# Anima-Lab/MaskDiT

Measured on AMD Instinct MI355X. Metric: training img/sec MaskDiT-XL/2 256 mask=0.5 bs=1024, higher is better.
Workload: dtype bf16; 1 GPU; DiT-XL/2 ImageNet256-latent [32x32x4], mask_ratio=0.5, mae_loss_coef=0.1, sample(moments)+class-dropout+fwd+bwd+grad-allreduce+AdamW+EMA, random-init (de-zeroed) weights; global_batch=1024, per_gpu_batch=1024, micro_batch=1024, accum=1, parallelism=dp1

## Files before the change

### include/maskdit_hip.h

```cpp
#ifndef MASKDIT_HIP_H
#define MASKDIT_HIP_H

#include <stdint.h>

#ifdef __cplusplus
extern "C" {
#endif

typedef void* mdt_stream_t;
typedef uint16_t mdt_bf16;

const char* mdt_last_error(void);
#define MDT_ABI_VERSION 4
int mdt_version(void);
int mdt_set_tuning(const char* key, int value);
int mdt_lds_poison(void* sink4, mdt_stream_t stream);
int mdt_nt8o_report(unsigned* abort_code, unsigned long long* stats16, int reset);
int mdt_nt8o_stamps(unsigned long long* host192);


enum mdt_epilogue {
  MDT_EPI_BF16 = 0,
  MDT_EPI_F32 = 1,
  MDT_EPI_GELU = 2,
// ... 8 lines not shown
  const mdt_bf16* B; int ldb;
  int M, N, K;
  const float* bias;
  int epi;
  mdt_bf16* out; int ldo;
  mdt_bf16* out2; int ldo2;
  float* outf; int ldof;
  const float* res; int ldres;
  const float* gate; int gate_ld; int rows_per_sample;
  const mdt_bf16* aux; int ldaux;
  int k_splits;
  float* colsum;
} mdt_gemm_nt_args;
int mdt_gemm_nt(const mdt_gemm_nt_args* a, mdt_stream_t stream);

typedef struct {
  const mdt_bf16* A; int lda;
  const mdt_bf16* B; int ldb;
  int M, N1, N2;
  float* C; int ldc;
  int n1_valid, n2_valid;
  int splits;
  float* colsum_a;
} mdt_gemm_tn_args;
int mdt_gemm_tn(const mdt_gemm_tn_args* a, mdt_stream_t stream);


int mdt_attn_fwd(const mdt_bf16* qkv, mdt_bf16* out, float* lse, int B, int L, int H, int hd, int L_valid,
                 mdt_stream_t stream);
int mdt_attn_bwd(const mdt_bf16* qkv, const mdt_bf16* out, const mdt_bf16* dout, const float* lse,
                 float* delta, mdt_bf16* dqkv, int B, int L, int H, int hd, int L_valid, mdt_stream_t stream);


int mdt_ln_modulate_fwd(const float* x, const float* shift, const float* scale, int mod_ld,
                        int rows_per_sample, mdt_bf16* xn, float* stats, int M, int D,
                        mdt_stream_t stream);
int mdt_ln_modulate_fwd_res(const float* xres, const mdt_bf16* y, const float* gate, int gate_ld, const float* shift,
                            const float* scale, int mod_ld, int rows_per_sample, float* x, mdt_bf16* xn, float* stats,
                            int M, int D, mdt_stream_t stream);
int mdt_ln_modulate_bwd(const mdt_bf16* dxn, const float* x, const float* stats, const float* scale,
                        int mod_ld, int rows_per_sample, float* dx, int accumulate, float* dshift,
                        float* dscale, int dmod_ld, int M, int D, mdt_stream_t stream);
int mdt_ln_modulate_bwd_gate(const mdt_bf16* dxn, const float* x, const float* stats, const float* scale,
                             int mod_ld, int rows_per_sample, float* dx, int accumulate, float* dshift,
                             float* dscale, int dmod_ld, int M, int D, const mdt_bf16* y, const float* gate,
                             int gate_ld, mdt_bf16* dys, float* dgate, int dgate_ld, float* dbias,
                             mdt_stream_t stream);
int mdt_gate_bwd(const float* dx, const mdt_bf16* y, const float* gate, int mod_ld,
// ... 204 lines not shown
```

### maskdit_amd/_lib.py

```python
from __future__ import annotations

import ctypes as C
import os
import subprocess

_HERE = os.path.dirname(os.path.abspath(__file__))
LIB_PATH = os.environ.get('MASKDIT_HIP_LIB') or os.path.join(_HERE, 'libmaskdit_hip.so')
CSRC = os.path.join(_HERE, 'csrc')

vp = C.c_void_p
i32 = C.c_int
i64 = C.c_long
f32 = C.c_float

EPI_BF16, EPI_F32, EPI_GELU, EPI_SILU, EPI_GATE_RES, EPI_DGELU, EPI_DSILU = range(7)


class GemmNTArgs(C.Structure):
    _fields_ = [('A', vp), ('lda', i32), ('B', vp), ('ldb', i32), ('M', i32), ('N', i32), ('K', i32),
                ('bias', vp), ('epi', i32), ('out', vp), ('ldo', i32), ('out2', vp), ('ldo2', i32),
                ('outf', vp), ('ldof', i32), ('res', vp), ('ldres', i32), ('gate', vp), ('gate_ld', i32),
                ('rows_per_sample', i32), ('aux', vp), ('ldaux', i32), ('k_splits', i32), ('colsum', vp)]


class GemmTNArgs(C.Structure):
    _fields_ = [('A', vp), ('lda', i32), ('B', vp), ('ldb', i32), ('M', i32), ('N1', i32), ('N2', i32),
                ('C', vp), ('ldc', i32), ('n1_valid', i32), ('n2_valid', i32), ('splits', i32), ('colsum_a', vp)]


class GemmF32Args(C.Structure):
    _fields_ = [('A', vp), ('lda', i64), ('B', vp), ('ldb', i64), ('b_kmajor', i32), ('M', i32), ('N', i32), ('K', i32),
                ('bias', vp), ('epi', i32), ('out', vp), ('ldo', i64), ('res', vp), ('ldres', i64), ('gate', vp),
                ('gate_ld', i64), ('rows_per_sample', i32), ('batch', i32), ('heads', i32),
                ('a_stride_b', i64), ('a_stride_h', i64), ('b_stride_b', i64), ('b_stride_h', i64),
                ('o_stride_b', i64), ('o_stride_h', i64)]


F32EPI_NONE, F32EPI_GELU, F32EPI_SILU, F32EPI_GATE_RES = range(4)


class GemmF32TNArgs(C.Structure):
    _fields_ = [('A', vp), ('lda', i64), ('B', vp), ('ldb', i64), ('M', i32), ('N1', i32), ('N2', i32), ('C', vp), ('ldc', i64),
                ('accumulate', i32), ('batch', i32), ('heads', i32),
                ('a_stride_b', i64), ('a_stride_h', i64), ('b_stride_b', i64), ('b_stride_h', i64),
                ('c_stride_b', i64), ('c_stride_h', i64), ('ws', vp), ('ws_floats', i64)]


_PROTOS = {
    'mdt_gemm_nt': [C.POINTER(GemmNTArgs)],
    'mdt_gemm_tn': [C.POINTER(GemmTNArgs)],
# ... 62 lines not shown
    'mdt_attn_f32_bwd': [vp, vp, vp, i64, vp, i32, i32, i32, i32],
    'mdt_ln_modulate_bwd_f32': [vp, vp, vp, i32, i32, vp, i32, vp, vp, i32, vp, i32, i32],
    'mdt_gate_bwd_f32': [vp, vp, vp, i32, i32, vp, vp, i32, i32, i32],
    'mdt_gate_res_f32': [vp, vp, vp, i32, i32, vp, i32, i32],
    'mdt_gelu_f32': [vp, vp, i64],
    'mdt_gelu_bwd_f32': [vp, vp, vp, i64],
    'mdt_silu_bwd_f32': [vp, vp, vp, i64],
}
_PLAIN = {
    'mdt_graph_begin': [vp],
    'mdt_graph_end': [vp, C.POINTER(vp)],
    'mdt_graph_launch': [vp, vp],
    'mdt_graph_destroy': [vp],
    'mdt_event_create': [C.POINTER(vp)],
    'mdt_event_record': [vp, vp],
    'mdt_event_elapsed_ms': [vp, vp, C.POINTER(f32)],
    'mdt_event_destroy': [vp],
    'mdt_set_tuning': [C.c_char_p, i32],
    'mdt_nt8o_report': [C.POINTER(C.c_uint32), C.POINTER(C.c_uint64), i32],
    'mdt_nt8o_stamps': [C.POINTER(C.c_uint64)],
    'mdt_attn_f32_ws_floats': [i32, i32, i32, i32],
    'mdt_gn_stats_ordered_ws_floats': [i32, i32],
    'mdt_gemm_f32_tn_ws_floats': [i32, i32, i32, i32],
    'mdt_colsum_f32_ws_floats': [i32, i32],
    'mdt_attn_f32_bwd_ws_floats': [i32, i32, i32, i32],
}
EXPORTED = sorted(list(_PROTOS) + list(_PLAIN) + ['mdt_last_error', 'mdt_version'])
ABI_VERSION = 4


class MaskDiTLibError(RuntimeError):
    pass


def source_hash() -> str:
    import glob
    import hashlib
    h = hashlib.sha256()
    root = os.path.dirname(os.path.abspath(__file__))
    files = sorted(glob.glob(os.path.join(root, 'csrc', '*.hip')) + glob.glob(os.path.join(root, 'csrc', '*.h')) +
                   glob.glob(os.path.join(root, '..', 'include', '*.h')))
    for f in files:
        h.update(os.path.basename(f).encode())
        h.update(open(f, 'rb').read())
    return h.hexdigest()[:16]

# ... 60 lines not shown
```

### maskdit_amd/csrc/gemm.hip

```cpp
#include "common.h"
#include "../../include/maskdit_hip.h"

#include "gemm_common.h"

#define BM 128
#define BN 128
#define BK 64
#define STAGE_BYTES 32768

__global__ __launch_bounds__(256, 2) void gemm_nt_kernel(NTParams p) {
  __shared__ __attribute__((aligned(16))) char smem[2 * STAGE_BYTES];
  const int tid = threadIdx.x;
  const int lane = tid & 63;
  const int wave = __builtin_amdgcn_readfirstlane(tid >> 6);
  const int wr = wave >> 1, wc = wave & 1;

  const int tiles_m = (p.M + BM - 1) / BM, tiles_n = p.N / BN;
  int tm, tn;
  tile_coords(xcd_remap(blockIdx.x, gridDim.x), tiles_m, tiles_n, tm, tn);
  const int m0 = tm * BM, n0 = tn * BN;

  const int lr = lane >> 3, cpos = lane & 7;
  const int gch = cpos ^ lr;
  const bf16* a_src[4];
// ... 259 lines not shown
      }
      if (w4 < 0.97 * w8 && w4 < 1e29) return launch_gemm_nt8(p, nf4, 1, (hipStream_t)stream);
      if (w8 < 1e29) return launch_gemm_nt8(p, nf8, 2, (hipStream_t)stream);
    }
    p.epi &= 0xff;
  }
  p.epi &= 0xff;
  int tiles = cdiv(a->M, BM) * (a->N / BN);
  int ks = 1;
  if (a->k_splits > 1) {
    MDT_REQUIRE(a->epi == MDT_EPI_F32 && a->out == nullptr, "gemm_nt: k_splits needs MDT_EPI_F32 without a bf16 output");
    MDT_REQUIRE(a->ldof == a->N, "gemm_nt: k_splits needs a dense outf (ldof == N)");
    ks = a->k_splits < a->K / BK ? a->k_splits : a->K / BK;
    if (hipMemsetAsync(a->outf, 0, sizeof(float) * (size_t)a->M * a->N, (hipStream_t)stream) != hipSuccess) {
      mdt_set_error("gemm_nt: clearing the split-K accumulator failed");
      return MDT_ERR_LAUNCH;
    }
  }
  p.k_splits = ks;
  hipLaunchKernelGGL(gemm_nt_kernel, dim3(tiles, ks), dim3(256), 0, (hipStream_t)stream, p);
  return mdt_check_launch("gemm_nt");
}

extern "C" int mdt_gemm_tn(const mdt_gemm_tn_args* a, mdt_stream_t stream) {
  MDT_REQUIRE(a && a->A && a->B && a->C, "gemm_tn: null operand");
  MDT_REQUIRE(a->M > 0 && a->M % BK == 0, "gemm_tn: M must be a positive multiple of 64");
  MDT_REQUIRE(a->N1 > 0 && a->N2 > 0, "gemm_tn: empty output");
  MDT_REQUIRE(a->lda % 8 == 0 && a->ldb % 8 == 0, "gemm_tn: lda/ldb must be multiples of 8");
  MDT_REQUIRE(a->lda >= cdiv(a->N1, BM) * BM && a->ldb >= cdiv(a->N2, BN) * BN,
              "gemm_tn: operand rows must be padded to a multiple of 128 columns");
  MDT_REQUIRE(((uintptr_t)a->A & 15) == 0 && ((uintptr_t)a->B & 15) == 0, "gemm_tn: operands must be 16-byte aligned");
  TNParams p;
  p.A = (const bf16*)a->A; p.lda = a->lda; p.B = (const bf16*)a->B; p.ldb = a->ldb;
  p.M = a->M; p.N1 = a->N1; p.N2 = a->N2; p.C = a->C; p.ldc = a->ldc;
  p.n1_valid = a->n1_valid > 0 ? a->n1_valid : a->N1;
  p.n2_valid = a->n2_valid > 0 ? a->n2_valid : a->N2;
  const int tn_variant = mdt_get_tuning_int(MDT_TUNE_GEMM_TN_VARIANT);
  if (tn_variant != 1 && p.n1_valid == a->N1 && p.n2_valid == a->N2 && a->N1 % 128 == 0 && a->N2 % 128 == 0 &&
      a->M % 32 == 0 && a->M >= 8192 && (long)a->N1 * a->N2 >= 256L * 1024) {
    int cs_done = 0;
    int rc = launch_gemm_tn8(p.A, p.lda, p.B, p.ldb, p.M, p.N1, p.N2, p.C, p.ldc, (hipStream_t)stream, a->colsum_a, &cs_done, a->splits);
    if (rc == MDT_OK && a->colsum_a && !cs_done) rc = mdt_colsum_bf16(a->A, a->lda, a->colsum_a, a->M, a->N1, stream);
    return rc;
  }
  if (a->colsum_a) {
    int rc = mdt_colsum_bf16(a->A, a->lda, a->colsum_a, a->M, a->N1, stream);
    if (rc != MDT_OK) return rc;
  }
  int tiles = cdiv(a->N1, BM) * cdiv(a->N2, BN);
  int ksteps = a->M / BK;
  int splits = a->splits;
  if (splits <= 0) {
    splits = 2048 / tiles;
    if (splits > ksteps / 8) splits = ksteps / 8;
    if (splits < 1) splits = 1;
  }
  if (splits > ksteps) splits = ksteps;
  p.ksteps_per_split = cdiv(ksteps, splits);
  splits = cdiv(ksteps, p.ksteps_per_split);
  p.splits = splits;
  hipLaunchKernelGGL(gemm_tn_kernel, dim3(tiles * splits), dim3(256), 0, (hipStream_t)stream, p);
  return mdt_check_launch("gemm_tn");
}
```

### maskdit_amd/csrc/gemm_common.h

```cpp
#pragma once
#include "common.h"
#include "../../include/maskdit_hip.h"

#define GROUP_M 8

struct NTParams {
  const bf16* A; int lda;
  const bf16* B; int ldb;
  int M, N, K;
  const float* bias;
  int epi;
  bf16* out; int ldo;
  bf16* out2; int ldo2;
  float* outf; int ldof;
  const float* res; int ldres;
  const float* gate; int gate_ld; int rows_per_sample;
  const bf16* aux; int ldaux;
  int k_splits;
  int group_m;
  float* colsum;
  int conv_ho_log2, conv_up, conv_c;
  float* gn_sums; int gn_cpg_log2;
};

// ... 129 lines not shown
  nt_load_bias<CW>(p, n, bias);
  nt_epilogue_prefetch<CW>(p, m, n, d);
  nt_epilogue_finish<CW>(p, m, n, v, bias, d, csum);
}

template <int CW> __device__ __forceinline__ void nt_colsum_flush(const NTParams& p, int n, float* csum, int lane) {
#pragma unroll
  for (int q = 0; q < CW; ++q) {
    float s = csum[q];
    s += __shfl_xor(s, 4, 64);
    s += __shfl_xor(s, 8, 64);
    s += __shfl_xor(s, 16, 64);
    s += __shfl_xor(s, 32, 64);
    if (lane < 4) atomic_add_f32(p.colsum + n + q, s);
  }
}

int launch_gemm_nt8(const NTParams& p, int nf, int wr, hipStream_t stream);
int nt8_num_cus();
int nt8_max_nf(int epi);
bool nt8o_eligible(const NTParams& p);
int launch_gemm_nt8o(const NTParams& p, int nl, int dbg, hipStream_t stream);
int launch_gemm_tn8(const bf16* A, int lda, const bf16* B, int ldb, int M, int N1, int N2, float* C, int ldc,
                    hipStream_t stream, float* colsum_a = nullptr, int* colsum_done = nullptr, int forced_splits = 0);
```

### maskdit_amd/csrc/gemm_tn8.hip

```cpp
#include "gemm_common.h"

template <int YF> struct TN8Cfg {
  static constexpr int NSLOT = YF == 6 ? 5 : 6;
  static constexpr int SLOT_BYTES = YF == 6 ? 28672 : 24576;
  static constexpr int TY = 32 * YF;
  static constexpr int UNROLL = YF == 6 ? 10 : 6;
};

__device__ __forceinline__ int tn8_swz(int r) { return ((r & 3) | (((r >> 3) & 1) << 2)) << 1; }
__device__ __forceinline__ int tn8_swz2(int r) { return (((r >> 1) & 1) | (((r >> 3) & 1) << 1)) << 1; }

struct TN8Params {
  const bf16* X; int ldx;
  const bf16* Y; int ldy;
  int NX, NY;
  float* C; int ldc;
  int swap;
  int slots_total;
  int slots_per_split;
  int tiles_x, tiles_y;
  float* colsum_x;
  int group_x;
  int dbg;
  int long_k, long_len;
};

template <int OFF> __device__ __forceinline__ bf16x4 tn8_tr_read(unsigned addr) {
  static_assert(OFF >= 0 && OFF < 65536, "ds offset field is 16 bits");
  short4_t v;
  asm volatile("ds_read_b64_tr_b16 %0, %1 offset:%2" : "=v"(v) : "v"(addr), "n"(OFF));
  return __builtin_bit_cast(bf16x4, v);
}

template <int N> __device__ __forceinline__ void tn8_wait() {
  static_assert(N >= 0 && N < 64, "vmcnt is 6 bits");
  asm volatile("; MDT_CHK hand_wait" ::: "memory");
  __builtin_amdgcn_s_waitcnt((N & 15) | (7 << 4) | (0 << 8) | ((N >> 4) << 14));
  asm volatile("" ::: "memory");
}

template <bool SWAP, int YF, bool FINE, bool CS>
__global__ __launch_bounds__(512, 2) void gemm_tn8_kernel(TN8Params p) {
  using Cfg = TN8Cfg<YF>;
  constexpr int NSLOT = Cfg::NSLOT, SLOT_BYTES = Cfg::SLOT_BYTES;
  constexpr int NSET = (NSLOT + 2) / 3;
  static_assert(2 * SLOT_BYTES + 1024 < 65536, "three slots per address set");
  __shared__ __attribute__((aligned(16))) char smem[NSLOT * SLOT_BYTES];
  const int tid = threadIdx.x;
  const int lane = tid & 63;
  const int wave = __builtin_amdgcn_readfirstlane(tid >> 6);
  const int wx = wave >> 1, wy = wave & 1;
  const bool mover2 = YF == 6 && wave < 4;

  const int tiles = p.tiles_x * p.tiles_y;
  int tile, s_begin, S;
  if (p.long_k == 0) {
    const int sid = xcd_remap(blockIdx.x, gridDim.x);
    const int split = sid / tiles;
    tile = sid - split * tiles;
    s_begin = split * p.slots_per_split;
    S = min(p.slots_per_split, p.slots_total - s_begin);
  } else {
    const int nlong = tiles * p.long_k;
    if ((int)blockIdx.x < nlong) {
      const int sid = xcd_remap(blockIdx.x, nlong);
      tile = sid % tiles;
      s_begin = (sid / tiles) * p.long_len;
      S = p.long_len;
    } else {
      tile = blockIdx.x - nlong;
      s_begin = p.long_k * p.long_len;
      S = p.slots_total - s_begin;
    }
  }
  int tx, ty;
  tile_coords(tile, p.tiles_x, p.tiles_y, tx, ty, p.group_x);
  const int x0 = tx * 256, y0 = ty * Cfg::TY;
  if (S <= 0) return;

  const int lr = lane >> 4, cpos = lane & 15;
  const int rloc = 4 * wave + lr;
  const int gch = cpos ^ tn8_swz(rloc);
  const int xc0 = min(x0 + gch * 8, p.NX - 8), xc1 = min(x0 + 128 + gch * 8, p.NX - 8);
  const int rloc2 = 8 * (wave & 3) + (lane >> 3);
  const char* const xu = (const char*)(p.X + (long)s_begin * 32 * p.ldx);
  const char* const yu = (const char*)(p.Y + (long)s_begin * 32 * p.ldy + y0);
  const unsigned x_lo0 = (unsigned)(rloc * p.ldx + xc0) * 2u, x_lo1 = (unsigned)(rloc * p.ldx + xc1) * 2u;
  const unsigned y_lo = (unsigned)(rloc * p.ldy + gch * 8) * 2u;
  const unsigned y_lo2 = (unsigned)(rloc2 * p.ldy + 128 + (((lane & 7) ^ tn8_swz2(rloc2)) << 3)) * 2u;
  const long x_step = 64L * p.ldx, y_step = 64L * p.ldy;
  char* const lds_w = smem + wave * 1024;

  auto issue = [&](int slot, int s, int parts = 15) {
// ... 182 lines not shown
#undef TN8_WAIT_PHASE
#undef TN8_BARRIER

  if (do_cs) {
    float* red = (float*)smem;
    asm volatile("s_waitcnt lgkmcnt(0)" ::: "memory");
    __builtin_amdgcn_s_barrier();
    asm volatile("" ::: "memory");
#pragma unroll
    for (int e = 0; e < 8; ++e) red[(cs_row * 16 + cs_c) * 8 + e] = cs_acc[e];
    asm volatile("s_waitcnt lgkmcnt(0)" ::: "memory");
    __builtin_amdgcn_s_barrier();
    asm volatile("" ::: "memory");
    if (tid < cs_n * 8) {
      float sum = 0.f;
      for (int r = 0; r < 32; ++r) sum += red[(r * 16 + (tid >> 3)) * 8 + (tid & 7)];
      const int col = x0 + (cs_begin + (tid >> 3)) * 8 + (tid & 7);
      if (col < p.NX) atomic_add_f32(p.colsum_x + col, sum);
    }
  }
#undef TN8_CS_READ
#undef TN8_CS_ADD

#pragma unroll
  for (int i = 0; i < 4; ++i)
#pragma unroll
    for (int j = 0; j < YF; ++j) {
      const int yb = y0 + (j < 4 ? wy * 64 + j * 16 : 128 + wy * 32 + (j - 4) * 16);
#pragma unroll
      for (int r = 0; r < 4; ++r) {
        if (!SWAP) {
          const int x = x0 + wx * 64 + i * 16 + g * 4 + r;
          const int y = yb + i16;
          if (x < p.NX) atomic_add_f32(p.C + (long)x * p.ldc + y, acc[i][j][r]);
        } else {
          const int x = x0 + wx * 64 + i * 16 + i16;
          const int y = yb + g * 4 + r;
          if (x < p.NX) atomic_add_f32(p.C + (long)y * p.ldc + x, acc[i][j][r]);
        }
      }
    }
}

int launch_gemm_tn8(const bf16* A, int lda, const bf16* B, int ldb, int M, int N1, int N2, float* C, int ldc,
                    hipStream_t stream, float* colsum_a, int* colsum_done, int forced_splits) {
  TN8Params p;
  auto x_waste = [](int nx) { return (double)(((nx + 255) / 256) * 256) / nx; };
  const int knob = mdt_get_tuning_int(MDT_TUNE_TN8_WIDE);
  int yf = 4;
  bool a_is_x;
  const bool b192 = knob != 1 && N2 % 192 == 0, a192 = knob != 1 && N1 % 192 == 0;
  if (b192 || a192) {
    yf = 6;
    a_is_x = b192 && (!a192 || x_waste(N1) <= x_waste(N2));
  } else {
    a_is_x = (N1 % 256 == 0) ? true : (N2 % 256 == 0) ? false : (N1 >= N2);
  }
  if (a_is_x) { p.X = A; p.ldx = lda; p.NX = N1; p.Y = B; p.ldy = ldb; p.NY = N2; p.swap = 0; }
  else { p.X = B; p.ldx = ldb; p.NX = N2; p.Y = A; p.ldy = lda; p.NY = N1; p.swap = 1; }
  p.C = C; p.ldc = ldc;
  p.tiles_x = (p.NX + 255) / 256;
  p.tiles_y = p.NY / (32 * yf);
  p.colsum_x = (colsum_a && a_is_x && p.tiles_y >= 2) ? colsum_a : nullptr;
  if (colsum_done) *colsum_done = p.colsum_x != nullptr;
  p.dbg = mdt_get_tuning_int(MDT_TUNE_TN8_DBG);
#ifndef MDT_EXPERIMENTS
  p.dbg &= ~7;
#endif
  p.group_x = ((p.dbg >> 4) & 15) ? ((p.dbg >> 4) & 15) : 2;
  const int nslot = yf == 6 ? TN8Cfg<6>::NSLOT : TN8Cfg<4>::NSLOT;
  p.slots_total = M / 32;
  const int tiles = p.tiles_x * p.tiles_y;
  const int cus = nt8_num_cus();
  int best = 1;
  double best_cost = 1e30;
  const double FIXED = 64.0;
  if (forced_splits > 0) best = forced_splits < p.slots_total / nslot ? forced_splits : (p.slots_total / nslot > 0 ? p.slots_total / nslot : 1);
  for (int sp = 1; sp <= 64 && forced_splits <= 0; ++sp) {
    if (sp > 1 && p.slots_total / sp < 32) break;
    const long blocks = (long)tiles * sp;
    const double cost = (double)((blocks + cus - 1) / cus) * ((double)((p.slots_total + sp - 1) / sp) + FIXED);
    if (cost < best_cost * 0.98) { best_cost = cost; best = sp; }
  }
  p.slots_per_split = (p.slots_total + best - 1) / best;
  if (p.slots_per_split < nslot) p.slots_per_split = nslot;
  int splits = (p.slots_total + p.slots_per_split - 1) / p.slots_per_split;
  if (splits > 1 && p.slots_total - (splits - 1) * p.slots_per_split < nslot) {
    p.slots_per_split = (p.slots_total + splits - 2) / (splits - 1);
    splits = (p.slots_total + p.slots_per_split - 1) / p.slots_per_split;
  }
  int grid_n = tiles * splits;
  p.long_k = p.long_len = 0;
  if (forced_splits <= 0 && !((p.dbg >> 8) & 1) && tiles < cus) {
    const int k = cus / tiles, R = cus - k * tiles;
    if (R > 0) {
      const int n = (tiles + R - 1) / R;
      const double TAIL = 1.35, S = (double)p.slots_total;
      int L = (int)((n * TAIL * S + (n - 1) * FIXED) / (1.0 + n * TAIL * k));
      if ((long)L * k > p.slots_total - 16) L = (p.slots_total - 16) / k;
      const int tail = p.slots_total - k * L;
      const double cost = fmax((double)L + FIXED, n * (TAIL * tail + FIXED));
      if (L >= 32 && tail >= 16 && tail >= nslot && cost < 0.97 * best_cost) {
        p.long_k = k;
        p.long_len = L;
        grid_n = tiles * k + tiles;
      }
    }
  }
  const dim3 grid(grid_n), block(512);
  const bool fine = (p.dbg & 8) == 0;
  const bool cs = p.colsum_x != nullptr;
#define TN8_LAUNCH2(SW, YFV, CSV) { if (fine) hipLaunchKernelGGL((gemm_tn8_kernel<SW, YFV, true, CSV>), grid, block, 0, stream, p); \
                                    else hipLaunchKernelGGL((gemm_tn8_kernel<SW, YFV, false, CSV>), grid, block, 0, stream, p); }
#define TN8_LAUNCH(SW, YFV) { if (cs && !SW) TN8_LAUNCH2(SW, YFV, (!SW)) else TN8_LAUNCH2(SW, YFV, false) }
  if (yf == 6) { if (p.swap) TN8_LAUNCH(true, 6) else TN8_LAUNCH(false, 6) }
  else { if (p.swap) TN8_LAUNCH(true, 4) else TN8_LAUNCH(false, 4) }
#undef TN8_LAUNCH2
#undef TN8_LAUNCH
  return mdt_check_launch("gemm_tn8");
}
```

### maskdit_amd/engine.py

```python
from __future__ import annotations

import ctypes as C
import os
import weakref
from dataclasses import dataclass
from typing import Callable, Dict, List, Optional, Tuple

import numpy as np
import torch

from . import _lib
from ._lib import (EPI_BF16, EPI_DGELU, EPI_DSILU, EPI_F32, EPI_GATE_RES, EPI_GELU, EPI_SILU, F32EPI_GATE_RES,
                   F32EPI_GELU, F32EPI_NONE, F32EPI_SILU, GemmF32Args, GemmF32TNArgs, GemmNTArgs, GemmTNArgs)

DEC_HIDDEN, DEC_DEPTH, DEC_HEADS = 512, 8, 16
MODEL_CONFIGS = {
    'DiT-H/2': (32, 1280, 2, 16), 'DiT-H/4': (32, 1280, 4, 16), 'DiT-H/8': (32, 1280, 8, 16),
    'DiT-XL/2': (28, 1152, 2, 16), 'DiT-XL/4': (28, 1152, 4, 16), 'DiT-XL/8': (28, 1152, 8, 16),
    'DiT-L/2': (24, 1024, 2, 16), 'DiT-L/4': (24, 1024, 4, 16), 'DiT-L/8': (24, 1024, 8, 16),
    'DiT-B/2': (12, 768, 2, 12), 'DiT-B/4': (12, 768, 4, 12), 'DiT-B/8': (12, 768, 8, 12),
    'DiT-S/2': (12, 384, 2, 6), 'DiT-S/4': (12, 384, 4, 6), 'DiT-S/8': (12, 384, 8, 6),
}
YPAD = 1024
LIVE_ENGINES: 'weakref.WeakSet' = weakref.WeakSet()
# ... 372 lines not shown
    return a


class PassPlan:

    def __init__(self, eng: Engine, B: int, masked: bool, train: bool, L: Optional[int], precision: str = 'bf16'):
        sp = eng.sp
        self.precision = precision
        self._eng_ref = weakref.ref(eng)
        self.B, self.masked, self.train = B, masked, train
        self.last_use = 0
        self.evict_hooks: List[Callable[[], None]] = []
        self.T = sp.T
        self.Lv = (L if L is not None else sp.T // 2) if masked else sp.T
        if not (1 <= self.Lv <= sp.T):
            raise ValueError(f'kept-token count {self.Lv} outside [1, {sp.T}]')
        self.L = _rup(self.Lv, 64)
        self.lv_arg = C.c_int(self.Lv)
        self.lv_attn = C.c_int(self.Lv if masked else 0)
        self.Bp = _rup(B, 64)
        self.buf: Dict[str, torch.Tensor] = {}
        self.fwd = Plan(eng.listing)
        self.bwd = Plan(eng.listing)
        self.gen = 0
        if train:
            eng.ensure_grad()
        if not reads_f32_arena(precision):
            self._build()
        elif train:
            self._build_f32_train()
        else:
            self._build_f32()

    @property
    def eng(self) -> Engine:
        e = self._eng_ref()
        if e is None:
            raise RuntimeError('maskdit_amd: this plan outlived its Engine (the model was deleted or re-bound)')
        return e

    @property
    def nbytes(self) -> int:
        return sum(t.numel() * t.element_size() for t in self.buf.values())

    @staticmethod
    def estimate_bytes(sp, B: int, masked: bool, train: bool, Lv: Optional[int]) -> int:
# ... 171 lines not shown
            self._block_bwd(f'model.blocks.{i}', 'e', i, xs_e[i], mod, dmod, sp.mod_off('enc', i), D, sp.heads, L, Me, dxe,
                            fuse_next=nxt, skip_first_gate=FUSE_LN_GATE, lvalid=self.lv_attn)
            self._slab(f'enc{i}')
            if f'ada_w_enc{i}' in groups:
                ada_group(f'ada_w_enc{i}', *groups[f'ada_w_enc{i}'])
        g.add('mdt_patch_embed_bwd', xin.data_ptr(), None, dxe.data_ptr(), ids32.data_ptr() if ids32 is not None else None,
              2 * T, Gf('model.x_embedder.proj.weight'), Gf('model.x_embedder.proj.bias'), B, sp.C, sp.R, sp.patch, L, D)
        dsc = self.f32('dsc', Bp, D)
        dc16 = self.b16('dc16', Bp, D)
        dh1 = self.b16('dh1', Bp, D)
        self._slab('ada_b')
        self._nt16(g, dmod16.data_ptr(), NM, WT('ada'), NM, B, D, NM, epi=EPI_F32, outf=dsc.data_ptr(), ldof=D,
                   k_splits=max(1, min(64, NM // 2048, 1024 // (((B + 127) // 128) * (D // 128)))))
        g.add('mdt_silu_bwd', dsc.data_ptr(), c.data_ptr(), dc16.data_ptr(), B * D)
        self._tn16(g, dc16.data_ptr(), D, lab16.data_ptr(), YPAD, Bp, D, YPAD, Gf('model.y_embedder.embedding_table.weight'),
                   sp.num_classes, n1v=D, n2v=sp.num_classes)
        self._tn16(g, dc16.data_ptr(), D, a1.data_ptr(), D, Bp, D, D, Gf('model.t_embedder.mlp.2.weight'), D)
        g.add('mdt_colsum_bf16', dc16.data_ptr(), D, Gf('model.t_embedder.mlp.2.bias'), B, D)
        self._nt16(g, dc16.data_ptr(), D, WT('model.t_embedder.mlp.2.weight'), D, B, D, D, epi=EPI_DSILU, out=dh1.data_ptr(), ldo=D,
                   aux=h1.data_ptr(), ldaux=D)
        self._tn16(g, dh1.data_ptr(), D, temb.data_ptr(), 256, Bp, D, 256, Gf('model.t_embedder.mlp.0.weight'), 256)
        g.add('mdt_colsum_bf16', dh1.data_ptr(), D, Gf('model.t_embedder.mlp.0.bias'), B, D)
        self._slab('misc')

    def _build_f32(self):
        self._fwd_f32(save=False)

    def _fwd_f32(self, save: bool):
        eng, sp, lay = self.eng, self.eng.sp, self.eng.lay
        B, T, D, Dd = self.B, self.T, sp.D, sp.Dd
        NM = sp.n_mod
        assert not self.masked
        if sp.num_classes % 4:
            raise NotImplementedError('fp32 path: num_classes must be a multiple of 4 (16-byte label rows)')
        if B * max(sp.heads, sp.dheads) > 65535:
            raise NotImplementedError('fp32 path: batch * heads must not exceed 65535 (one grid row per (sample, head))')
        Pf, Pp = self.Pf, eng.P.data_ptr()
        f = self.fwd
        xin, cn, lab, _, Fx = self._io()
        temb, a1 = self.f32('temb', B, 256), self.f32('a1', B, D)
        c_t, c, sc = self.f32('c_t', B, D), self.f32('c', B, D), self.f32('sc', B, D)
        mod = self.f32('mod', B, NM)
        f.add('mdt_timestep_embed_f32', cn.data_ptr(), temb.data_ptr(), 256, B, 256)
        if save:
            h1 = self.f32('h1', B, D)
            self._g32(temb, 256, Pf('model.t_embedder.mlp.0.weight'), 256, B, D, 256, h1, D, bias=Pf('model.t_embedder.mlp.0.bias'))
# ... 222 lines not shown
        f.add('mdt_ln_modulate_f32', x_in.data_ptr(), sh1, sc1, NM, rows, xn.data_ptr(), M, W)
        self._g32(xn, W, Pf(p + 'attn.qkv.weight'), W, M, 3 * W, W, qkv, 3 * W, bias=Pf(p + 'attn.qkv.bias'))
        f.add('mdt_attn_f32', qkv.data_ptr(), ao.data_ptr(), S, B, rows, heads, hd)
        branch(ao, W, 'attn.proj', x_in, g1, f'fa_{s}', xmid)
        f.add('mdt_ln_modulate_f32', xmid.data_ptr(), sh2, sc2, NM, rows, xn.data_ptr(), M, W)
        self._g32(xn, W, Pf(p + 'mlp.fc1.weight'), W, M, 4 * W, W, h, 4 * W, bias=Pf(p + 'mlp.fc1.bias'),
                  epi=F32EPI_NONE if save else F32EPI_GELU)
        act = h
        if save:
            act = self.f32(f'act_{tag}', M, 4 * W)
            f.add('mdt_gelu_f32', h.data_ptr(), act.data_ptr(), M * 4 * W)
        branch(act, 4 * W, 'mlp.fc2', xmid, g2, f'fm_{s}', xout)
        return xout

    def _k(self, obj):
        self.fwd.keep.append(obj)
        return obj

    def _nt16(self, to: Plan, *a, **kw):
        to.add('mdt_gemm_nt', C.byref(self._k(_nt(*a, **kw))))

    def _tn16(self, to: Plan, *a, **kw):
        to.add('mdt_gemm_tn', C.byref(self._k(_tn(*a, **kw))))

    def _slab(self, name):
        ref = self._eng_ref
        lo, hi = self.eng.lay.slabs[name]

        def cb():
            eng = ref()
            if eng is not None and eng.grad_slab_hook is not None:
                eng.grad_slab_hook(name, lo, hi)

        self.bwd.add_callback(cb)

    def _block_fwd(self, prefix, tag, i, x_in, mod, moff, W, heads, rows, M, lvalid=0, pending=None, defer_out=False):
        f = self.fwd
        NM = self.eng.sp.n_mod
        hd = W // heads
        B = self.B
        s = f'{tag}{i}' if self.train else f'{tag}'
        p, Pf, Wp = prefix + '.', self.Pf, self.Wp
        mp = mod.data_ptr()
        sh1, sc1, g1, sh2, sc2, g2 = (mp + 4 * (moff + k * W) for k in range(6))
        xn1, st1 = self.b16(f'xn1_{s}', M, W), self.f32(f'st1_{s}', M, 2)
        qkv = self.b16(f'qkv_{s}', M, 3 * W)
# ... 109 lines not shown
```

### maskdit_amd/ops.py

```python
from __future__ import annotations

import ctypes as C

import torch

from . import _lib
from ._lib import (EPI_BF16, EPI_DGELU, EPI_DSILU, EPI_F32, EPI_GATE_RES, EPI_GELU, EPI_SILU, F32EPI_GATE_RES,
                   F32EPI_GELU, F32EPI_NONE, F32EPI_SILU, GemmF32Args, GemmNTArgs, GemmTNArgs, call)


def stream_ptr() -> int:
    return torch.cuda.current_stream().cuda_stream


def p(t):
    return None if t is None else t.data_ptr()


def _need(t, dtype, name):
    if t.dtype != dtype or not t.is_cuda or not t.is_contiguous():
        raise ValueError(f'{name}: expected contiguous CUDA {dtype}, got {t.dtype} cuda={t.is_cuda} contig={t.is_contiguous()}')


def gemm_nt(A, Bw, bias=None, epi=EPI_BF16, out=None, out2=None, outf=None, res=None, gate=None, gate_ld=0,
# ... 4 lines not shown
    N, K = Bw.shape[0], A.shape[1]
    a = GemmNTArgs()
    a.A, a.lda, a.B, a.ldb, a.M, a.N, a.K = p(A), A.stride(0), p(Bw), Bw.stride(0), M, N, K
    a.bias, a.epi = p(bias), epi
    if epi in (EPI_BF16, EPI_GELU, EPI_SILU, EPI_GATE_RES, EPI_DGELU, EPI_DSILU) and out is None and not (
            no_out and epi in (EPI_GELU, EPI_SILU, EPI_GATE_RES)):
        out = torch.empty(A.shape[0], N, device=A.device, dtype=torch.bfloat16)
    if epi in (EPI_GELU, EPI_SILU) and out2 is None:
        out2 = torch.empty(A.shape[0], N, device=A.device, dtype=torch.bfloat16)
    if epi in (EPI_F32, EPI_GATE_RES) and outf is None:
        outf = torch.empty(A.shape[0], N, device=A.device, dtype=torch.float32)
    a.out, a.ldo = p(out), (out.stride(0) if out is not None else 0)
    a.out2, a.ldo2 = p(out2), (out2.stride(0) if out2 is not None else 0)
    a.outf, a.ldof = p(outf), (outf.stride(0) if outf is not None else 0)
    a.res, a.ldres = p(res), (res.stride(0) if res is not None else 0)
    a.gate, a.gate_ld, a.rows_per_sample = p(gate), gate_ld, rows_per_sample
    a.aux, a.ldaux = p(aux), (aux.stride(0) if aux is not None else 0)
    a.k_splits = k_splits
    a.colsum = p(colsum)
    call('mdt_gemm_nt', C.byref(a), stream_ptr())
    return out, out2, outf


def gemm_tn(A, Bm, Cout, n1_valid=0, n2_valid=0, splits=0, N1=None, N2=None, colsum_a=None):
    _need(A, torch.bfloat16, 'A')
    _need(Bm, torch.bfloat16, 'B')
    a = GemmTNArgs()
    a.A, a.lda, a.B, a.ldb = p(A), A.stride(0), p(Bm), Bm.stride(0)
    a.M, a.N1, a.N2 = A.shape[0], (N1 or A.shape[1]), (N2 or Bm.shape[1])
    a.C, a.ldc, a.n1_valid, a.n2_valid, a.splits = p(Cout), Cout.stride(0), n1_valid, n2_valid, splits
    a.colsum_a = p(colsum_a) if colsum_a is not None else None
    call('mdt_gemm_tn', C.byref(a), stream_ptr())
    return Cout


def attn_fwd(qkv, B, L, H, hd, L_valid=0):
    out = torch.empty(B * L, H * hd, device=qkv.device, dtype=torch.bfloat16)
    lse = torch.empty(B * H * L, device=qkv.device, dtype=torch.float32)
    call('mdt_attn_fwd', p(qkv), p(out), p(lse), B, L, H, hd, L_valid, stream_ptr())
    return out, lse


def attn_bwd(qkv, out, dout, lse, B, L, H, hd, L_valid=0):
    dqkv = torch.empty_like(qkv)
    delta = torch.empty_like(lse)
    call('mdt_attn_bwd', p(qkv), p(out), p(dout), p(lse), p(delta), p(dqkv), B, L, H, hd, L_valid, stream_ptr())
    return dqkv


def ln_modulate_fwd(x, shift, scale, mod_ld, rows_per_sample):
    M, D = x.shape
    xn = torch.empty(M, D, device=x.device, dtype=torch.bfloat16)
    stats = torch.empty(M, 2, device=x.device, dtype=torch.float32)
    call('mdt_ln_modulate_fwd', p(x), p(shift), p(scale), mod_ld, rows_per_sample, p(xn), p(stats), M, D, stream_ptr())
    return xn, stats

# ... 99 lines not shown
```

Measured before the change: 2285 img/s.

## Reduce split-K TN GEMM partials via workspace slabs and a fold kernel

Split-K weight-gradient GEMMs (tn8) can now write each split's accumulator tile to a per-slab float workspace instead of accumulating directly into C. A separate fold kernel then sums the slabs and adds the result into C. The engine allocates one shared workspace sized by a new ws_floats query and attaches it to every TN GEMM call. This is meant to remove the cost of contended atomic/read-modify-write accumulation into C across splits, at the price of extra workspace memory traffic and an additional kernel launch per GEMM.

Measured after the change: 2285 img/s. No clear change (-0.0%).

```diff
diff --git a/include/maskdit_hip.h b/include/maskdit_hip.h
--- a/include/maskdit_hip.h
+++ b/include/maskdit_hip.h
@@ -54,8 +54,10 @@
   int n1_valid, n2_valid;
   int splits;
   float* colsum_a;
+  float* ws; long long ws_floats;
 } mdt_gemm_tn_args;
 int mdt_gemm_tn(const mdt_gemm_tn_args* a, mdt_stream_t stream);
+long long mdt_gemm_tn_ws_floats(int M, int N1, int N2);
 
 
 int mdt_attn_fwd(const mdt_bf16* qkv, mdt_bf16* out, float* lse, int B, int L, int H, int hd, int L_valid,
diff --git a/maskdit_amd/_lib.py b/maskdit_amd/_lib.py
--- a/maskdit_amd/_lib.py
+++ b/maskdit_amd/_lib.py
@@ -25,7 +25,8 @@
 
 class GemmTNArgs(C.Structure):
     _fields_ = [('A', vp), ('lda', i32), ('B', vp), ('ldb', i32), ('M', i32), ('N1', i32), ('N2', i32),
-                ('C', vp), ('ldc', i32), ('n1_valid', i32), ('n2_valid', i32), ('splits', i32), ('colsum_a', vp)]
+                ('C', vp), ('ldc', i32), ('n1_valid', i32), ('n2_valid', i32), ('splits', i32), ('colsum_a', vp),
+                ('ws', vp), ('ws_floats', C.c_longlong)]
 
 
 class GemmF32Args(C.Structure):
@@ -134,6 +135,7 @@
     'mdt_attn_f32_ws_floats': [i32, i32, i32, i32],
     'mdt_gn_stats_ordered_ws_floats': [i32, i32],
     'mdt_gemm_f32_tn_ws_floats': [i32, i32, i32, i32],
+    'mdt_gemm_tn_ws_floats': [i32, i32, i32],
     'mdt_colsum_f32_ws_floats': [i32, i32],
     'mdt_attn_f32_bwd_ws_floats': [i32, i32, i32, i32],
 }
diff --git a/maskdit_amd/csrc/gemm.hip b/maskdit_amd/csrc/gemm.hip
--- a/maskdit_amd/csrc/gemm.hip
+++ b/maskdit_amd/csrc/gemm.hip
@@ -305,6 +305,13 @@
   return mdt_check_launch("gemm_nt");
 }
 
+static bool tn8_shape(int M, int N1, int N2) {
+  return mdt_get_tuning_int(MDT_TUNE_GEMM_TN_VARIANT) != 1 && N1 > 0 && N2 > 0 && N1 % 128 == 0 && N2 % 128 == 0 && M % 32 == 0 &&
+         M >= 8192 && (long)N1 * N2 >= 256L * 1024;
+}
+
+extern "C" long long mdt_gemm_tn_ws_floats(int M, int N1, int N2) { return tn8_shape(M, N1, N2) ? tn8_ws_floats(M, N1, N2) : 0; }
+
 extern "C" int mdt_gemm_tn(const mdt_gemm_tn_args* a, mdt_stream_t stream) {
   MDT_REQUIRE(a && a->A && a->B && a->C, "gemm_tn: null operand");
   MDT_REQUIRE(a->M > 0 && a->M % BK == 0, "gemm_tn: M must be a positive multiple of 64");
@@ -313,16 +320,20 @@
   MDT_REQUIRE(a->lda >= cdiv(a->N1, BM) * BM && a->ldb >= cdiv(a->N2, BN) * BN,
               "gemm_tn: operand rows must be padded to a multiple of 128 columns");
   MDT_REQUIRE(((uintptr_t)a->A & 15) == 0 && ((uintptr_t)a->B & 15) == 0, "gemm_tn: operands must be 16-byte aligned");
+  const bool to_tn8 = (a->n1_valid <= 0 || a->n1_valid == a->N1) && (a->n2_valid <= 0 || a->n2_valid == a->N2) &&
+                      tn8_shape(a->M, a->N1, a->N2);
+  MDT_REQUIRE(!a->ws || !to_tn8 ||
+                  (((uintptr_t)a->ws & 15) == 0 && a->ws_floats >= mdt_gemm_tn_ws_floats(a->M, a->N1, a->N2)),
+              "gemm_tn: workspace unaligned or smaller than mdt_gemm_tn_ws_floats()");
   TNParams p;
   p.A = (const bf16*)a->A; p.lda = a->lda; p.B = (const bf16*)a->B; p.ldb = a->ldb;
   p.M = a->M; p.N1 = a->N1; p.N2 = a->N2; p.C = a->C; p.ldc = a->ldc;
   p.n1_valid = a->n1_valid > 0 ? a->n1_valid : a->N1;
   p.n2_valid = a->n2_valid > 0 ? a->n2_valid : a->N2;
-  const int tn_variant = mdt_get_tuning_int(MDT_TUNE_GEMM_TN_VARIANT);
-  if (tn_variant != 1 && p.n1_valid == a->N1 && p.n2_valid == a->N2 && a->N1 % 128 == 0 && a->N2 % 128 == 0 &&
-      a->M % 32 == 0 && a->M >= 8192 && (long)a->N1 * a->N2 >= 256L * 1024) {
+  if (to_tn8) {
     int cs_done = 0;
-    int rc = launch_gemm_tn8(p.A, p.lda, p.B, p.ldb, p.M, p.N1, p.N2, p.C, p.ldc, (hipStream_t)stream, a->colsum_a, &cs_done, a->splits);
+    int rc = launch_gemm_tn8(p.A, p.lda, p.B, p.ldb, p.M, p.N1, p.N2, p.C, p.ldc, (hipStream_t)stream, a->colsum_a, &cs_done, a->splits,
+                             a->ws, a->ws_floats);
     if (rc == MDT_OK && a->colsum_a && !cs_done) rc = mdt_colsum_bf16(a->A, a->lda, a->colsum_a, a->M, a->N1, stream);
     return rc;
   }
diff --git a/maskdit_amd/csrc/gemm_common.h b/maskdit_amd/csrc/gemm_common.h
--- a/maskdit_amd/csrc/gemm_common.h
+++ b/maskdit_amd/csrc/gemm_common.h
@@ -175,4 +175,6 @@
 bool nt8o_eligible(const NTParams& p);
 int launch_gemm_nt8o(const NTParams& p, int nl, int dbg, hipStream_t stream);
 int launch_gemm_tn8(const bf16* A, int lda, const bf16* B, int ldb, int M, int N1, int N2, float* C, int ldc,
-                    hipStream_t stream, float* colsum_a = nullptr, int* colsum_done = nullptr, int forced_splits = 0);
+                    hipStream_t stream, float* colsum_a = nullptr, int* colsum_done = nullptr, int forced_splits = 0,
+                    float* ws = nullptr, long ws_floats = 0);
+long tn8_ws_floats(int M, int N1, int N2);
diff --git a/maskdit_amd/csrc/gemm_tn8.hip b/maskdit_amd/csrc/gemm_tn8.hip
--- a/maskdit_amd/csrc/gemm_tn8.hip
+++ b/maskdit_amd/csrc/gemm_tn8.hip
@@ -23,6 +23,8 @@
   int group_x;
   int dbg;
   int long_k, long_len;
+  float* ws;
+  int nslab;
 };
 
 template <int OFF> __device__ __forceinline__ bf16x4 tn8_tr_read(unsigned addr) {
@@ -39,7 +41,7 @@
   asm volatile("" ::: "memory");
 }
 
-template <bool SWAP, int YF, bool FINE, bool CS>
+template <bool SWAP, int YF, bool FINE, bool CS, bool WS>
 __global__ __launch_bounds__(512, 2) void gemm_tn8_kernel(TN8Params p) {
   using Cfg = TN8Cfg<YF>;
   constexpr int NSLOT = Cfg::NSLOT, SLOT_BYTES = Cfg::SLOT_BYTES;
@@ -53,11 +55,12 @@
   const bool mover2 = YF == 6 && wave < 4;
 
   const int tiles = p.tiles_x * p.tiles_y;
-  int tile, s_begin, S;
+  int tile, s_begin, S, slab;
   if (p.long_k == 0) {
     const int sid = xcd_remap(blockIdx.x, gridDim.x);
     const int split = sid / tiles;
     tile = sid - split * tiles;
+    slab = split;
     s_begin = split * p.slots_per_split;
     S = min(p.slots_per_split, p.slots_total - s_begin);
   } else {
@@ -65,10 +68,12 @@
     if ((int)blockIdx.x < nlong) {
       const int sid = xcd_remap(blockIdx.x, nlong);
       tile = sid % tiles;
-      s_begin = (sid / tiles) * p.long_len;
+      slab = sid / tiles;
+      s_begin = slab * p.long_len;
       S = p.long_len;
     } else {
       tile = blockIdx.x - nlong;
+      slab = p.long_k;
       s_begin = p.long_k * p.long_len;
       S = p.slots_total - s_begin;
     }
@@ -297,6 +302,14 @@
 #undef TN8_CS_READ
 #undef TN8_CS_ADD
 
+  if constexpr (WS) {
+    f32x4* dst = (f32x4*)p.ws + (((long)slab * tiles + tile) * 8 + wave) * (4 * YF * 64) + lane;
+#pragma unroll
+    for (int i = 0; i < 4; ++i)
+#pragma unroll
+      for (int j = 0; j < YF; ++j) dst[(i * YF + j) * 64] = acc[i][j];
+    return;
+  }
 #pragma unroll
   for (int i = 0; i < 4; ++i)
 #pragma unroll
@@ -317,9 +330,43 @@
     }
 }
 
-int launch_gemm_tn8(const bf16* A, int lda, const bf16* B, int ldb, int M, int N1, int N2, float* C, int ldc,
-                    hipStream_t stream, float* colsum_a, int* colsum_done, int forced_splits) {
-  TN8Params p;
+template <bool SWAP, int YF>
+__global__ __launch_bounds__(256) void tn8_fold_kernel(TN8Params p) {
+  const int tiles = p.tiles_x * p.tiles_y;
+  const long vecs = (long)tiles * (8 * 4 * YF * 64);
+  const long idx = (long)blockIdx.x * 256 + threadIdx.x;
+  if (idx >= vecs) return;
+  const int lane = (int)idx & 63, i16 = lane & 15, g = lane >> 4;
+  int q = (int)(idx >> 6);
+  const int j = q % YF;
+  q /= YF;
+  const int i = q & 3, wave = (q >> 2) & 7, tile = q >> 5;
+  const int wx = wave >> 1, wy = wave & 1;
+  int tx, ty;
+  tile_coords(tile, p.tiles_x, p.tiles_y, tx, ty, p.group_x);
+  const f32x4* src = (const f32x4*)p.ws + idx;
+  f32x4 sum = src[0];
+#pragma unroll 4
+  for (int s = 1; s < p.nslab; ++s) {
+    const f32x4 v = src[(long)s * vecs];
+#pragma unroll
+    for (int r = 0; r < 4; ++r) sum[r] += v[r];
+  }
+  const int yb = ty * (32 * YF) + (j < 4 ? wy * 64 + j * 16 : 128 + wy * 32 + (j - 4) * 16);
+  const int xb = tx * 256 + wx * 64 + i * 16;
+#pragma unroll
+  for (int r = 0; r < 4; ++r) {
+    if (!SWAP) {
+      const int x = xb + g * 4 + r, y = yb + i16;
+      if (x < p.NX) p.C[(long)x * p.ldc + y] += sum[r];
+    } else {
+      const int x = xb + i16, y = yb + g * 4 + r;
+      if (x < p.NX) p.C[(long)y * p.ldc + x] += sum[r];
+    }
+  }
+}
+
+static int tn8_plan(TN8Params& p, int M, int N1, int N2, int forced_splits, int cus, bool* a_is_x_out) {
   auto x_waste = [](int nx) { return (double)(((nx + 255) / 256) * 256) / nx; };
   const int knob = mdt_get_tuning_int(MDT_TUNE_TN8_WIDE);
   int yf = 4;
@@ -331,13 +378,11 @@
   } else {
     a_is_x = (N1 % 256 == 0) ? true : (N2 % 256 == 0) ? false : (N1 >= N2);
   }
-  if (a_is_x) { p.X = A; p.ldx = lda; p.NX = N1; p.Y = B; p.ldy = ldb; p.NY = N2; p.swap = 0; }
-  else { p.X = B; p.ldx = ldb; p.NX = N2; p.Y = A; p.ldy = lda; p.NY = N1; p.swap = 1; }
-  p.C = C; p.ldc = ldc;
+  *a_is_x_out = a_is_x;
+  if (a_is_x) { p.NX = N1; p.NY = N2; p.swap = 0; }
+  else { p.NX = N2; p.NY = N1; p.swap = 1; }
   p.tiles_x = (p.NX + 255) / 256;
   p.tiles_y = p.NY / (32 * yf);
-  p.colsum_x = (colsum_a && a_is_x && p.tiles_y >= 2) ? colsum_a : nullptr;
-  if (colsum_done) *colsum_done = p.colsum_x != nullptr;
   p.dbg = mdt_get_tuning_int(MDT_TUNE_TN8_DBG);
 #ifndef MDT_EXPERIMENTS
   p.dbg &= ~7;
@@ -346,7 +391,6 @@
   const int nslot = yf == 6 ? TN8Cfg<6>::NSLOT : TN8Cfg<4>::NSLOT;
   p.slots_total = M / 32;
   const int tiles = p.tiles_x * p.tiles_y;
-  const int cus = nt8_num_cus();
   int best = 1;
   double best_cost = 1e30;
   const double FIXED = 64.0;
@@ -364,7 +408,7 @@
     p.slots_per_split = (p.slots_total + splits - 2) / (splits - 1);
     splits = (p.slots_total + p.slots_per_split - 1) / p.slots_per_split;
   }
-  int grid_n = tiles * splits;
+  p.nslab = splits;
   p.long_k = p.long_len = 0;
   if (forced_splits <= 0 && !((p.dbg >> 8) & 1) && tiles < cus) {
     const int k = cus / tiles, R = cus - k * tiles;
@@ -378,19 +422,68 @@
       if (L >= 32 && tail >= 16 && tail >= nslot && cost < 0.97 * best_cost) {
         p.long_k = k;
         p.long_len = L;
-        grid_n = tiles * k + tiles;
+        p.nslab = k + 1;
       }
     }
   }
+  return yf;
+}
+
+static long tn8_slab_floats(const TN8Params& p, int yf) { return (long)p.tiles_x * p.tiles_y * 256 * 32 * yf; }
+
+static bool tn8_wants_ws(const TN8Params& p, int cus, bool ignore_off_switch) {
+  if (p.nslab < 2 || (p.dbg & 8) || (!ignore_off_switch && ((p.dbg >> 9) & 1))) return false;
+  if ((p.dbg >> 10) & 1) return true;
+  return p.long_k == 0 && p.tiles_x * p.tiles_y * p.nslab <= cus && p.slots_per_split <= 256 && p.nslab <= 8;
+}
+
+long tn8_ws_floats(int M, int N1, int N2) {
+  TN8Params p;
+  bool a_is_x;
+  const int cus = nt8_num_cus();
+  const int yf = tn8_plan(p, M, N1, N2, 0, cus, &a_is_x);
+  return tn8_wants_ws(p, cus, true) ? p.nslab * tn8_slab_floats(p, yf) : 0L;
+}
+
+int launch_gemm_tn8(const bf16* A, int lda, const bf16* B, int ldb, int M, int N1, int N2, float* C, int ldc,
+                    hipStream_t stream, float* colsum_a, int* colsum_done, int forced_splits, float* ws, long ws_floats) {
+  TN8Params p;
+  const int cus = nt8_num_cus();
+  bool a_is_x;
+  const int yf = tn8_plan(p, M, N1, N2, forced_splits, cus, &a_is_x);
+  const bool partial = ws && (forced_splits > 0 ? p.nslab >= 2 && !(p.dbg & 8) && !((p.dbg >> 9) & 1) : tn8_wants_ws(p, cus, false));
+  if (partial && p.nslab * tn8_slab_floats(p, yf) > ws_floats) {
+    mdt_set_error("gemm_tn: workspace smaller than this partition needs (forced splits, or \"nt8_max_cus\" changed since mdt_gemm_tn_ws_floats())");
+    return MDT_ERR_ARG;
+  }
+  if (a_is_x) { p.X = A; p.ldx = lda; p.Y = B; p.ldy = ldb; }
+  else { p.X = B; p.ldx = ldb; p.Y = A; p.ldy = lda; }
+  p.C = C; p.ldc = ldc;
+  p.ws = partial ? ws : nullptr;
+  p.colsum_x = (colsum_a && a_is_x && p.tiles_y >= 2) ? colsum_a : nullptr;
+  if (colsum_done) *colsum_done = p.colsum_x != nullptr;
+  const int tiles = p.tiles_x * p.tiles_y;
+  const int grid_n = p.long_k ? tiles * p.long_k + tiles : tiles * p.nslab;
   const dim3 grid(grid_n), block(512);
   const bool fine = (p.dbg & 8) == 0;
   const bool cs = p.colsum_x != nullptr;
-#define TN8_LAUNCH2(SW, YFV, CSV) { if (fine) hipLaunchKernelGGL((gemm_tn8_kernel<SW, YFV, true, CSV>), grid, block, 0, stream, p); \
-                                    else hipLaunchKernelGGL((gemm_tn8_kernel<SW, YFV, false, CSV>), grid, block, 0, stream, p); }
+#define TN8_LAUNCH2(SW, YFV, CSV) { if (partial) hipLaunchKernelGGL((gemm_tn8_kernel<SW, YFV, true, CSV, true>), grid, block, 0, stream, p); \
+                                    else if (fine) hipLaunchKernelGGL((gemm_tn8_kernel<SW, YFV, true, CSV, false>), grid, block, 0, stream, p); \
+                                    else hipLaunchKernelGGL((gemm_tn8_kernel<SW, YFV, false, CSV, false>), grid, block, 0, stream, p); }
 #define TN8_LAUNCH(SW, YFV) { if (cs && !SW) TN8_LAUNCH2(SW, YFV, (!SW)) else TN8_LAUNCH2(SW, YFV, false) }
   if (yf == 6) { if (p.swap) TN8_LAUNCH(true, 6) else TN8_LAUNCH(false, 6) }
   else { if (p.swap) TN8_LAUNCH(true, 4) else TN8_LAUNCH(false, 4) }
 #undef TN8_LAUNCH2
 #undef TN8_LAUNCH
-  return mdt_check_launch("gemm_tn8");
-}
+  int rc = mdt_check_launch("gemm_tn8");
+  if (rc != MDT_OK || !partial) return rc;
+  const dim3 fgrid((unsigned)(tiles * 8 * yf));
+  if (yf == 6) {
+    if (p.swap) hipLaunchKernelGGL((tn8_fold_kernel<true, 6>), fgrid, dim3(256), 0, stream, p);
+    else hipLaunchKernelGGL((tn8_fold_kernel<false, 6>), fgrid, dim3(256), 0, stream, p);
+  } else {
+    if (p.swap) hipLaunchKernelGGL((tn8_fold_kernel<true, 4>), fgrid, dim3(256), 0, stream, p);
+    else hipLaunchKernelGGL((tn8_fold_kernel<false, 4>), fgrid, dim3(256), 0, stream, p);
+  }
+  return mdt_check_launch("gemm_tn8 (fold)");
+}
diff --git a/maskdit_amd/engine.py b/maskdit_amd/engine.py
--- a/maskdit_amd/engine.py
+++ b/maskdit_amd/engine.py
@@ -418,6 +418,7 @@
         self.buf: Dict[str, torch.Tensor] = {}
         self.fwd = Plan(eng.listing)
         self.bwd = Plan(eng.listing)
+        self._tn_args: List[GemmTNArgs] = []
         self.gen = 0
         if train:
             eng.ensure_grad()
@@ -635,6 +636,7 @@
         self._tn16(g, dh1.data_ptr(), D, temb.data_ptr(), 256, Bp, D, 256, Gf('model.t_embedder.mlp.0.weight'), 256)
         g.add('mdt_colsum_bf16', dh1.data_ptr(), D, Gf('model.t_embedder.mlp.0.bias'), B, D)
         self._slab('misc')
+        self._tn_workspace()
 
     def _build_f32(self):
         self._fwd_f32(save=False)
@@ -903,6 +905,15 @@
 
     def _tn16(self, to: Plan, *a, **kw):
         to.add('mdt_gemm_tn', C.byref(self._k(_tn(*a, **kw))))
+        self._tn_args.append(self.fwd.keep[-1])
+
+    def _tn_workspace(self):
+        L = _lib.lib()
+        n = max((int(L.mdt_gemm_tn_ws_floats(a.M, a.N1, a.N2)) for a in self._tn_args if not (a.n1_valid or a.n2_valid)), default=0)
+        if n:
+            ws = self.f32('tn_ws', n)
+            for a in self._tn_args:
+                a.ws, a.ws_floats = ws.data_ptr(), n
 
     def _slab(self, name):
         ref = self._eng_ref
diff --git a/maskdit_amd/ops.py b/maskdit_amd/ops.py
--- a/maskdit_amd/ops.py
+++ b/maskdit_amd/ops.py
@@ -50,7 +50,7 @@
     return out, out2, outf
 
 
-def gemm_tn(A, Bm, Cout, n1_valid=0, n2_valid=0, splits=0, N1=None, N2=None, colsum_a=None):
+def gemm_tn(A, Bm, Cout, n1_valid=0, n2_valid=0, splits=0, N1=None, N2=None, colsum_a=None, ws=None):
     _need(A, torch.bfloat16, 'A')
     _need(Bm, torch.bfloat16, 'B')
     a = GemmTNArgs()
@@ -58,8 +58,16 @@
     a.M, a.N1, a.N2 = A.shape[0], (N1 or A.shape[1]), (N2 or Bm.shape[1])
     a.C, a.ldc, a.n1_valid, a.n2_valid, a.splits = p(Cout), Cout.stride(0), n1_valid, n2_valid, splits
     a.colsum_a = p(colsum_a) if colsum_a is not None else None
+    if ws is not None:
+        if ws.dtype != torch.float32 or not ws.is_cuda:
+            raise ValueError('ws: expected a CUDA float32 tensor')
+        a.ws, a.ws_floats = p(ws), ws.numel()
     call('mdt_gemm_tn', C.byref(a), stream_ptr())
     return Cout
+
+
+def gemm_tn_ws_floats(M, N1, N2):
+    return int(_lib.lib().mdt_gemm_tn_ws_floats(M, N1, N2))
 
 
 def attn_fwd(qkv, B, L, H, hd, L_valid=0):
```
